# iacopo97/Multimodal-SAM-Adapter

Hardware: AMD Instinct MI355X
Metric: images/sec encoder fwd @1024x1024 RGB+LiDAR ViT-L (higher is better)
Workload: dtype split-operand MFMA: fp16 hi + e5m2 cross terms (h8c / h8 planes, ViT / interaction / up-conv GEMMs) fp16 hi/lo pairs x3 (TwinConvNeXt: f3 planes) and bf16 hi/lo x3 (neck, head); attention blocks with the rel-pos terms fused: every contraction on one fp16 MFMA (q, k, v, P rounded to fp16) in the bloc

## Files before the change

### include/mmsa.h

```cpp
#ifndef MMSA_H
#define MMSA_H
#include <stddef.h>
#include <stdint.h>
#ifdef __cplusplus
extern "C" {
#endif

#ifdef MMSA_BUILDING_LIBRARY
typedef hipStream_t mmsa_stream_t;
#else
typedef void* mmsa_stream_t;
#endif

#include "mmsa_version.h"
int mmsa_version(void);
const char* mmsa_last_error(void);

int mmsa_debug_poison_lds(unsigned pattern, mmsa_stream_t stream);
int mmsa_event_create(void** ev);
int mmsa_event_record(void* ev, mmsa_stream_t stream);
int mmsa_event_elapsed_ms(void* start, void* stop, float* ms);
int mmsa_event_destroy(void* ev);

enum { MMSA_ACT_NONE = 0, MMSA_ACT_GELU = 1, MMSA_ACT_RELU = 2, MMSA_ACT_RELU6 = 3, MMSA_ACT_HSWISH = 4, MMSA_ACT_SIGMOID = 5 };
// ... 16 lines not shown
int mmsa_msda_fused(const float* value, const int64_t* spatial_shapes, const int64_t* level_start_index,
                    const float* raw, long ldraw, const float* ref_points, float* out, long ldo,
                    uint16_t* out_planes, long ldop , int out_fmt , int batch,
                    int spatial_size, int num_heads, int channels, int num_levels, int num_query, int num_point,
                    float* clamp_max , mmsa_stream_t stream);

int mmsa_msda_fused_planes(const uint16_t* value_planes, long ldvp, int lo_bytes, const int64_t* spatial_shapes, const int64_t* level_start_index,
                           const float* raw, long ldraw, const float* ref_points, float* out, long ldo,
                           uint16_t* out_planes, long ldop, int out_fmt, int batch,
                           int spatial_size, int num_heads, int channels, int num_levels, int num_query, int num_point,
                           float* clamp_max, mmsa_stream_t stream);

int mmsa_rowstats_finalize(const float* rowstats, int rows, int strips, int D, float eps, float* mean_rstd, mmsa_stream_t stream);

int mmsa_zero_bytes(void* p, size_t bytes, mmsa_stream_t stream);
int mmsa_gemm_split3(const float* A, const uint16_t* Ap, long lda, long strideA,
                     const uint16_t* Wp, long strideW,
                     const float* bias, long strideBias, const float* colscale, const float* resid, long ldr,
                     long strideR, int resid_mod, float beta, float* C, long ldc, long strideC,
                     uint16_t* Cp, long ldcp, long strideCp, int M, int N, int K,
                     int batch, int act, float alpha, int out_mode, int ps_H, int ps_W, int ps_C, int fmt, int cp_fmt,
                     int max_grid, float* rowstats_out, const float* rownorm_mean_rstd, const float* rownorm_colsum, int flavour,
                     float* clamp_max , mmsa_stream_t stream);

int mmsa_convnext_mlp_fused(const uint16_t* Ap, long lda, long strideA, const uint16_t* W1p, long strideW1, const uint16_t* W2p,
                            long strideW2, const float* b1, const float* b2, const float* gamma, float* x, long ldx, long strideX,
                            int M, int C, int batch, int max_grid, int fmt,
                            float* clamp_max , mmsa_stream_t stream);

int mmsa_split_planes(const float* src, long ld, int rows, int cols, int cols_pad, uint16_t* planes, int kind,
                      float* clamp_max , mmsa_stream_t stream);

int mmsa_attention(const float* qkv, long ldq, const float* qkv_bias, const float* rp, float* out, long ldo, int B,
                   int H, int W, int heads, int head_dim, int window_size, float scale, mmsa_stream_t stream);
int mmsa_attention_planes(const uint16_t* qkv_planes, long ldq, const uint16_t* bias_planes, const float* rp,
                          uint16_t* out_planes, long ldo, int B, int H, int W, int heads, int head_dim,
                          int window_size, float scale, int out_fmt ,
                          int v_fmt ,
                          float* max_abs_logit , mmsa_stream_t stream);

int mmsa_relpos_bias(const float* qkv, long ldq, const float* Rh, const float* Rw, float* rp, int B, int H, int W,
                     int heads, int head_dim, int window_size, mmsa_stream_t stream);
int mmsa_relpos_bias_planes(const uint16_t* qkv_planes, long ldq, const float* Rh, const float* Rw,
                            float* rp, int B, int H, int W, int heads, int head_dim, int window_size, mmsa_stream_t stream);

int mmsa_layernorm_rows(const float* x, long ldx, const float* w, const float* b, float eps, float* y, long ldy,
// ... 108 lines not shown
```

### include/mmsa_version.h

```cpp
#ifndef MMSA_VERSION_H
#define MMSA_VERSION_H
#define MMSA_ABI_VERSION 109
#endif
```

### multimodal-sam-adapter_amd/csrc/gemm_split3.hip

```cpp
#include "common.h"

struct GemmArgs {
  const float* A; const unsigned short* Ap; long lda; long strideA;
  const unsigned short* Wp; long strideW;
  const float* bias; long strideBias;
  const float* colscale;
  const float* resid; long ldr; long strideR; int resid_mod; float beta;
  float* C; long ldc; long strideC;
  unsigned short* Cp; long ldcp; long strideCp;
  int M, N, K;
  int act; float alpha;
  int out_mode; int ps_H, ps_W, ps_C;
  int cp_fmt;
  float* clamp_max;
};

#define BM 128
#define BN 128
#define BK 32
#define PLANE_BYTES (4 * 128 * 16)
#define STAGE_BYTES (4 * PLANE_BYTES)

template <bool AP, bool GEN, bool F16 = false>
__global__ __launch_bounds__(256) void gemm_split3_kernel(GemmArgs a) {
// ... 202 lines not shown
        for (int r = 0; r < 4; ++r) {
          if (n + r < a.N) {
            float x = v[r];
            if (resid) x += a.beta * resid[rrow * a.ldr + dcol + r];
            if (C) C[drow * a.ldc + dcol + r] = x;
            if (Cp) { clamp_see1(cw_, x); store_planes1(Cp + drow * a.ldcp, dcol + r, x, MMSA_CP_AT(a.cp_fmt, dcol + r)); }
          }
        }
      }
    }
  }
  if (Cp) clamp_report(a.clamp_max, cw_, MMSA_CP_SPLIT(a.cp_fmt) ? MMSA_H8_MAX : mmsa_clamp_limit(MMSA_CP_BASE(a.cp_fmt)));
}

int mmsa_gemm_v2_launch(const unsigned short* Ap, long lda, long strideA,
                        const unsigned short* Wp, long strideW,
                        const float* bias, long strideBias, const float* colscale,
                        const float* resid, long ldr, long strideR, int resid_mod, float beta,
                        float* C, long ldc, long strideC,
                        unsigned short* Cp, long ldcp, long strideCp,
                        int M, int N, int K, int batch, int act, float alpha,
                        int out_mode, int ps_H, int ps_W, int ps_C, int fmt, int cp_fmt, int max_grid, hipStream_t stream,
                        float* rs_out, const float* rn_mr, const float* rn_cs, int flavour, float* clamp_max);

__global__ __launch_bounds__(256) void gemm_tiny_kernel(GemmArgs a, int ncg) {
  const int lane = threadIdx.x & 63;
  const long wv = (long)blockIdx.x * 4 + (threadIdx.x >> 6);
  const long per_b = (long)a.M * ncg;
  const int bz = blockIdx.y;
  if (wv >= per_b) return;
  const int m = (int)(wv / ncg), n0 = (int)(wv - (long)m * ncg) * 8;
  const float* A = a.A + (long)bz * a.strideA + (long)m * a.lda;
  const unsigned short* Wp = a.Wp + (long)bz * a.strideW;
  float acc[8];
#pragma unroll
  for (int j = 0; j < 8; ++j) acc[j] = 0.f;
  for (int k = lane * 4; k < a.K; k += 256) {
    const float4 x = *reinterpret_cast<const float4*>(A + k);
    const int ko = ilv(k);
#pragma unroll
    for (int j = 0; j < 8; ++j) {
      const int n = min(n0 + j, a.N - 1);
      const unsigned short* wr = Wp + (long)n * 2 * a.K + ko;
      const uint2 h = *reinterpret_cast<const uint2*>(wr), l = *reinterpret_cast<const uint2*>(wr + 32);
      const float w0 = __uint_as_float(h.x << 16) + __uint_as_float(l.x << 16);
      const float w1 = __uint_as_float(h.x & 0xFFFF0000u) + __uint_as_float(l.x & 0xFFFF0000u);
// ... 71 lines not shown
  a.bias = bias; a.strideBias = strideBias; a.colscale = colscale;
  a.resid = resid; a.ldr = ldr; a.strideR = strideR; a.resid_mod = resid_mod; a.beta = beta;
  a.C = C; a.ldc = C ? ldc : 0; a.strideC = strideC;
  a.Cp = Cp; a.ldcp = Cp ? ldcp : 0; a.strideCp = strideCp;
  a.M = M; a.N = N; a.K = K; a.act = act; a.alpha = alpha;
  a.out_mode = out_mode; a.ps_H = ps_H; a.ps_W = ps_W; a.ps_C = ps_C; a.cp_fmt = cp_fmt;
  a.clamp_max = clamp_max;
  const bool force_v1 = MMSA_KNOB("MMSA_GEMM_V1", 0) != 0;
  const bool narrow = false;
  const bool no_tiny = MMSA_KNOB("MMSA_GEMM_NO_TINY", 0) != 0;
  if (!ap && !Cp && out_mode == 0 && resid_mod <= 0 && (N <= 64 || K <= 64) && M <= 16384 && !no_tiny && !extras && fmt == MMSA_FMT_B3) {
    const int ncg = cdiv(N, 8);
    hipLaunchKernelGGL(gemm_tiny_kernel, dim3(cdiv((long)M * ncg, 4), batch), dim3(256), 0, stream, a, ncg);
    MMSA_CHECK_LAUNCH("gemm_split3(tiny)");
    return MMSA_OK;
  }
  if (ap && (fmt != MMSA_FMT_B3 || (M >= 128 && !force_v1 && !narrow))) {
    return mmsa_gemm_v2_launch(Ap, lda, strideA, Wp, strideW, bias, strideBias, colscale, resid, ldr, strideR,
                               resid_mod, beta, C, ldc, strideC, Cp, ldcp, strideCp, M, N, K, batch, act, alpha,
                               out_mode, ps_H, ps_W, ps_C, fmt, cp_fmt, max_grid, stream, rs_out, rn_mr, rn_cs, flavour, clamp_max);
  }
  MMSA_CHECK_ARG(!extras, "gemm_split3: this shape is not routed to the LDS-DMA kernel, which alone writes row statistics / normalises rows");
  MMSA_CHECK_ARG(!cp_h8c, "gemm_split3: h8c output planes are written by the LDS-DMA kernel only (activation planes in, M >= 128)");
  dim3 grid(cdiv(N, BN), cdiv(M, BM), batch);
  const bool gen = out_mode != 0 || resid_mod > 0;
  if (ap) {
    if (gen) hipLaunchKernelGGL((gemm_split3_kernel<true, true>), grid, dim3(256), 2 * STAGE_BYTES, stream, a);
    else hipLaunchKernelGGL((gemm_split3_kernel<true, false>), grid, dim3(256), 2 * STAGE_BYTES, stream, a);
  } else if (fmt == MMSA_FMT_F3) {
    if (gen) hipLaunchKernelGGL((gemm_split3_kernel<false, true, true>), grid, dim3(256), 2 * STAGE_BYTES, stream, a);
    else hipLaunchKernelGGL((gemm_split3_kernel<false, false, true>), grid, dim3(256), 2 * STAGE_BYTES, stream, a);
  } else {
    if (gen) hipLaunchKernelGGL((gemm_split3_kernel<false, true>), grid, dim3(256), 2 * STAGE_BYTES, stream, a);
    else hipLaunchKernelGGL((gemm_split3_kernel<false, false>), grid, dim3(256), 2 * STAGE_BYTES, stream, a);
  }
  MMSA_CHECK_LAUNCH("gemm_split3");
  return MMSA_OK;
}

__global__ void split_planes_kernel(const float* __restrict__ src, long ld, int rows, int cols, int cols_pad,
                                    unsigned short* __restrict__ out, int kind, float* __restrict__ clamp_max) {
  const long total = (long)rows * cols_pad;
  float cw_ = 0.f;
  for (long i = (long)blockIdx.x * blockDim.x + threadIdx.x; i < total; i += (long)gridDim.x * blockDim.x) {
    const int r = (int)(i / cols_pad), c = (int)(i % cols_pad);
    const float x = c < cols ? src[(long)r * ld + c] : 0.f;
// ... 38 lines not shown
```

### multimodal-sam-adapter_amd/csrc/gemm_stream.hip

```cpp
#include "gemm_v2_shared.h"

struct GemmStreamArgs {
  const unsigned short* Ap; long lda;
  const unsigned short* Wp;
  const float* bias; const float* colscale; float alpha;
  const float* resid; long ldr; float beta;
  float* C; long ldc;
  unsigned short* Cp; long ldcp; int cp_fmt;
  int M, act;
  float* clamp_max;
};

#define GS_WROW(K_) ((K_) * 4 + 16)

template <int NT, int KS, bool F16, bool RES>
__global__ __launch_bounds__(512, 1) void gemm_stream_kernel(GemmStreamArgs a) {
  constexpr int N = NT * 16, K = KS * 32;
  extern __shared__ __attribute__((aligned(16))) unsigned char smem[];
  const int tid = threadIdx.x, lane = tid & 63;
  const int wave = __builtin_amdgcn_readfirstlane(tid >> 6);
  const int l15 = lane & 15, g = lane >> 4;

  {
    constexpr int PIECES = N * KS * 8;
    const unsigned char* wsrc = reinterpret_cast<const unsigned char*>(a.Wp);
    for (int p = tid; p < PIECES; p += 512) {
      const int n = p / (KS * 8), q = p - n * (KS * 8);
      *reinterpret_cast<uint4*>(smem + n * GS_WROW(K) + q * 16) = *reinterpret_cast<const uint4*>(wsrc + (long)n * (K * 4) + q * 16);
    }
  }
  if (tid < N) {
    float* cvl = reinterpret_cast<float*>(smem + N * GS_WROW(K));
    cvl[tid] = a.bias ? a.bias[tid] : 0.f;
    cvl[N + tid] = (a.colscale ? a.colscale[tid] : 1.f) * a.alpha;
  }
  __syncthreads();

  const int nblk = (a.M + 15) >> 4;
  const int stride = gridDim.x * 8;
  int blk = blockIdx.x * 8 + wave;
  if (blk >= nblk) return;
  const unsigned char* Ab = reinterpret_cast<const unsigned char*>(a.Ap);
  const long ldaB = a.lda * 2;
  const unsigned woff0 = (unsigned)(l15 * GS_WROW(K) + g * 16);

  uint4 fa[2][KS][2];
  auto load_block = [&](int b_, uint4 (&f)[KS][2]) {
    const int row = min(b_ * 16 + l15, a.M - 1);
    const unsigned char* rp = Ab + (long)row * ldaB + g * 16;
#pragma unroll
    for (int ks = 0; ks < KS; ++ks) {
      f[ks][0] = *reinterpret_cast<const uint4*>(rp + ks * 128);
      f[ks][1] = *reinterpret_cast<const uint4*>(rp + ks * 128 + 64);
    }
  };
  const int cp_base = MMSA_CP_BASE(a.cp_fmt);
  const bool act_on = a.act != ACT_NONE;
  const float act_hi = a.act == ACT_RELU6 ? 6.0f : INFINITY;
  float cw_ = 0.f;
  const float* colv = reinterpret_cast<const float*>(smem + N * GS_WROW(K)) + 4 * g;

  auto compute_store = [&](int b_, const uint4 (&f)[KS][2]) {
    const int m = b_ * 16 + l15;
    float4 rr[NT];
    if constexpr (RES) {
      const float* rrow = a.resid + (long)min(m, a.M - 1) * a.ldr + 4 * g;
#pragma unroll
      for (int nt = 0; nt < NT; ++nt) rr[nt] = *reinterpret_cast<const float4*>(rrow + nt * 16);
    }
    f32x4 acc[NT];
#pragma unroll
    for (int nt = 0; nt < NT; ++nt) acc[nt] = (f32x4){0.f, 0.f, 0.f, 0.f};
    unsigned woff = woff0;
    asm volatile("" : "+v"(woff));
    const unsigned char* wl_ = smem + woff;
#pragma unroll
    for (int ks = 0; ks < KS; ++ks) {
#pragma unroll
      for (int nt = 0; nt < NT; ++nt) {
        const uint4 wh = *reinterpret_cast<const uint4*>(wl_ + nt * 16 * GS_WROW(K) + ks * 128);
        const uint4 wl = *reinterpret_cast<const uint4*>(wl_ + nt * 16 * GS_WROW(K) + ks * 128 + 64);
        if constexpr (F16) {
          acc[nt] = __builtin_amdgcn_mfma_f32_16x16x32_f16(__builtin_bit_cast(f16x8, wl), __builtin_bit_cast(f16x8, f[ks][0]), acc[nt], 0, 0, 0);
          acc[nt] = __builtin_amdgcn_mfma_f32_16x16x32_f16(__builtin_bit_cast(f16x8, wh), __builtin_bit_cast(f16x8, f[ks][1]), acc[nt], 0, 0, 0);
          acc[nt] = __builtin_amdgcn_mfma_f32_16x16x32_f16(__builtin_bit_cast(f16x8, wh), __builtin_bit_cast(f16x8, f[ks][0]), acc[nt], 0, 0, 0);
        } else {
          acc[nt] = __builtin_amdgcn_mfma_f32_16x16x32_bf16(__builtin_bit_cast(bf16x8, wl), __builtin_bit_cast(bf16x8, f[ks][0]), acc[nt], 0, 0, 0);
          acc[nt] = __builtin_amdgcn_mfma_f32_16x16x32_bf16(__builtin_bit_cast(bf16x8, wh), __builtin_bit_cast(bf16x8, f[ks][1]), acc[nt], 0, 0, 0);
          acc[nt] = __builtin_amdgcn_mfma_f32_16x16x32_bf16(__builtin_bit_cast(bf16x8, wh), __builtin_bit_cast(bf16x8, f[ks][0]), acc[nt], 0, 0, 0);
        }
      }
    }
    if (m < a.M) {
#pragma unroll
      for (int nt = 0; nt < NT; ++nt) {
        const int n = nt * 16 + 4 * g;
        const float4 bv = *reinterpret_cast<const float4*>(colv + 16 * nt), cv = *reinterpret_cast<const float4*>(colv + N + 16 * nt);
        float4 o = make_float4(acc[nt][0] + bv.x, acc[nt][1] + bv.y, acc[nt][2] + bv.z, acc[nt][3] + bv.w);
        if (act_on) { o.x = fminf(fmaxf(o.x, 0.0f), act_hi); o.y = fminf(fmaxf(o.y, 0.0f), act_hi); o.z = fminf(fmaxf(o.z, 0.0f), act_hi); o.w = fminf(fmaxf(o.w, 0.0f), act_hi); }
        o.x *= cv.x; o.y *= cv.y; o.z *= cv.z; o.w *= cv.w;
        if constexpr (RES) { o.x += a.beta * rr[nt].x; o.y += a.beta * rr[nt].y; o.z += a.beta * rr[nt].z; o.w += a.beta * rr[nt].w; }
        if (a.C) *reinterpret_cast<float4*>(a.C + (long)m * a.ldc + n) = o;
        if (a.Cp) {
          clamp_see(cw_, o);
          store_planes4(a.Cp + (long)m * a.ldcp, n, o, cp_base);
        }
      }
    }
  };

  const int lastb = nblk - 1;
  load_block(blk, fa[0]);
#pragma unroll 1
  for (;;) {
    const int nb1 = blk + stride;
    load_block(min(nb1, lastb), fa[1]);
    compute_store(blk, fa[0]);
    if (nb1 >= nblk) break;
    const int nb2 = nb1 + stride;
    load_block(min(nb2, lastb), fa[0]);
    compute_store(nb1, fa[1]);
    if (nb2 >= nblk) break;
    blk = nb2;
  }
  if (a.Cp) clamp_report(a.clamp_max, cw_, mmsa_clamp_limit(cp_base));
}

int mmsa_gemm_stream_try(const unsigned short* Ap, long lda, const unsigned short* Wp, const float* bias, const float* colscale, const float* resid, long ldr, float beta,
                         float* C, long ldc, unsigned short* Cp, long ldcp, int M, int N, int K, int batch, int act, float alpha, int out_mode, int resid_mod,
                         int fmt, int cp_fmt, int max_grid, const float* rs_out, const float* rn_mr, int flavour, float* clamp_max, hipStream_t stream) {
#ifndef MMSA_GEMM_STREAM_DEFAULT
#define MMSA_GEMM_STREAM_DEFAULT 1
#endif
  if (MMSA_KNOB("MMSA_GEMM_STREAM", MMSA_GEMM_STREAM_DEFAULT) == 0 || flavour != 0) return 0;
  if (!(fmt == MMSA_FMT_B3 || fmt == MMSA_FMT_F3) || batch != 1 || out_mode != 0 || resid_mod > 0 || rs_out || rn_mr) return 0;
  if (!((N == 96 && K == 192) || (N == 192 && K == 96)) || M < 16384) return 0;
  if (!(act == ACT_NONE || act == ACT_RELU || act == ACT_RELU6)) return 0;
  if (Cp && (MMSA_CP_SPLIT(cp_fmt) != 0 || !(MMSA_CP_BASE(cp_fmt) == MMSA_FMT_B3 || MMSA_CP_BASE(cp_fmt) == MMSA_FMT_F3))) return 0;
  const uintptr_t al = (uintptr_t)Ap | (uintptr_t)Wp | (uintptr_t)bias | (uintptr_t)colscale | (uintptr_t)resid | (uintptr_t)C | (uintptr_t)Cp;
  if ((al & 15) || (lda & 7) || (C && (ldc & 3)) || (resid && (ldr & 3)) || (Cp && (ldcp & 7)) || lda < 2L * K || (Cp && ldcp < 2L * N)) return 0;
  GemmStreamArgs a;
  a.Ap = Ap; a.lda = lda; a.Wp = Wp; a.bias = bias; a.colscale = colscale; a.alpha = alpha; a.resid = resid; a.ldr = ldr; a.beta = beta;
  a.C = C; a.ldc = ldc; a.Cp = Cp; a.ldcp = ldcp; a.cp_fmt = cp_fmt; a.M = M; a.act = act; a.clamp_max = clamp_max;
  static MmsaPerDevice per_dev_ = {};
  const int num_cus = mmsa_per_device(per_dev_, [] {
#define GS_ATTR(NT_, KS_, F_) (void)hipFuncSetAttribute((const void*)gemm_stream_kernel<NT_, KS_, F_, false>, hipFuncAttributeMaxDynamicSharedMemorySize, (NT_) * 16 * GS_WROW((KS_) * 32) + (NT_) * 16 * 8); \
                              (void)hipFuncSetAttribute((const void*)gemm_stream_kernel<NT_, KS_, F_, true>, hipFuncAttributeMaxDynamicSharedMemorySize, (NT_) * 16 * GS_WROW((KS_) * 32) + (NT_) * 16 * 8);
    GS_ATTR(6, 6, false) GS_ATTR(6, 6, true) GS_ATTR(12, 3, false) GS_ATTR(12, 3, true)
#undef GS_ATTR
  });
  const int cus = (max_grid > 0 && max_grid < num_cus) ? max_grid : num_cus;
  const int nblk = (M + 15) / 16;
  const int grid = nblk / 8 < cus ? (nblk + 7) / 8 : cus;
  const int lds = N * GS_WROW(K) + N * 8;
  const bool f16 = fmt == MMSA_FMT_F3;
#define GS_LAUNCH(NT_, KS_)                                                                                                   \
  { if (f16 && resid) hipLaunchKernelGGL((gemm_stream_kernel<NT_, KS_, true, true>), dim3(grid), dim3(512), lds, stream, a);      \
    else if (f16) hipLaunchKernelGGL((gemm_stream_kernel<NT_, KS_, true, false>), dim3(grid), dim3(512), lds, stream, a);          \
    else if (resid) hipLaunchKernelGGL((gemm_stream_kernel<NT_, KS_, false, true>), dim3(grid), dim3(512), lds, stream, a);        \
    else hipLaunchKernelGGL((gemm_stream_kernel<NT_, KS_, false, false>), dim3(grid), dim3(512), lds, stream, a); }
  if (N == 96 && K == 192) GS_LAUNCH(6, 6)
  else GS_LAUNCH(12, 3)
#undef GS_LAUNCH
  MMSA_CHECK_LAUNCH("gemm_split3(stream)");
  return 1;
}
```

### multimodal-sam-adapter_amd/csrc/gemm_v2.hip

```cpp
#include "common.h"
#include "gemm_v2_shared.h"
template <bool GEN, int ACT, bool PP, int NW, int FMT>
__global__ __launch_bounds__(NW * 64, NW == 4 ? 2 : 1) void gemm_v2_kernel(GemmV2Args a) {
  static_assert(NW == 8 || (NW == 4 && !PP), "4-wave workgroups run the in-phase main loop");
  static_assert(FMT == MMSA_FMT_B3 || (PP && NW == 8), "the h8 and f3 operand formats run on the ping-pong kernel");
  constexpr bool EPI_UNROLL = ACT >= 0;
  constexpr int V2_BM = NW * 32;
  constexpr int V2_A_BYTES = V2_BM * 128;
  constexpr int V2_STAGE = V2_A_BYTES + V2_W_BYTES;
  constexpr int V2_NST = NW == 8 ? 3 : 2;
  constexpr int WROWS = V2_BN / NW;
  constexpr int NDMA = 4 + WROWS / 8;
  extern __shared__ __attribute__((aligned(16))) unsigned char smem[];
  const int tid = threadIdx.x;
  const int lane = tid & 63;
  const int wave = __builtin_amdgcn_readfirstlane(tid >> 6);
  const int wm = wave >> 1, wn = wave & 1;
  const int grp = wave >> 2;
  const int l15 = lane & 15, g = lane >> 4;
  const int K = a.K;
  const int nk = K / V2_BK;

  const int G = gridDim.x;
  int rb = blockIdx.x;
// ... 403 lines not shown
    const int st_cur = st == 0 ? V2_NST - 1 : st - 1;

    if (V2_DBG(a) == 2 || V2_DBG(a) == 5 || V2_DBG(a) >= 64) { tile += G; continue; }
#define EPI_STAGING_BASE (smem + st_cur * V2_STAGE)
#include "gemm_v2_epilogue.inc"
    if constexpr (PP) {
      asm volatile("s_waitcnt lgkmcnt(0)" ::: "memory");
      __builtin_amdgcn_s_barrier();
    }
    tile += G;
  }
  CLK_SAMPLE(2)
#undef K_STEP
#undef K_STEP_PP
#undef K_STEP_PP_FAST
#undef PP_WAIT
#undef PP_PIECE
#undef MFMA_CHUNK
#undef MFMA_FP8_ALL
}

int mmsa_gemm_h8c_dispatch(const GemmV2Args& a, int grid, bool gen, int act, hipStream_t stream);
int mmsa_gemm_h8c_w8_dispatch(const GemmV2Args& a, int grid, bool gen, int act, hipStream_t stream);
int mmsa_gemm_stream_try(const unsigned short* Ap, long lda, const unsigned short* Wp, const float* bias, const float* colscale, const float* resid, long ldr, float beta,
                         float* C, long ldc, unsigned short* Cp, long ldcp, int M, int N, int K, int batch, int act, float alpha, int out_mode, int resid_mod,
                         int fmt, int cp_fmt, int max_grid, const float* rs_out, const float* rn_mr, int flavour, float* clamp_max, hipStream_t stream);
int mmsa_gemm_h8c4_dispatch(const GemmV2Args& a, int grid, hipStream_t stream);

int mmsa_gemm_v2_launch(const unsigned short* Ap, long lda, long strideA,
                        const unsigned short* Wp, long strideW,
                        const float* bias, long strideBias, const float* colscale,
                        const float* resid, long ldr, long strideR, int resid_mod, float beta,
                        float* C, long ldc, long strideC,
                        unsigned short* Cp, long ldcp, long strideCp,
                        int M, int N, int K, int batch, int act, float alpha,
                        int out_mode, int ps_H, int ps_W, int ps_C, int fmt, int cp_fmt, int max_grid, hipStream_t stream,
                        float* rs_out, const float* rn_mr, const float* rn_cs, int flavour, float* clamp_max) {
  {
    const int rc_ = mmsa_gemm_stream_try(Ap, lda, Wp, bias, colscale, resid, ldr, beta, C, ldc, Cp, ldcp, M, N, K, batch, act, alpha, out_mode, resid_mod, fmt, cp_fmt,
                                         max_grid, rs_out, rn_mr, flavour, clamp_max, stream);
    if (rc_ != 0) return rc_ < 0 ? rc_ : MMSA_OK;
  }
  GemmV2Args a;
  a.clamp_max = clamp_max;
  MMSA_CHECK_ARG(!rs_out || (C && out_mode == 0 && resid_mod <= 0 && act == ACT_NONE && (N & 63) == 0 && (ldc & 3) == 0 && (!resid || (ldr & 3) == 0) && (!Cp || (ldcp & 3) == 0)),
                 "gemm(v2): row statistics need a plain fp32 output, no activation, N %% 64 == 0 (N=%d)", N);
  MMSA_CHECK_ARG(!rn_mr || (rn_cs && !resid && out_mode == 0 && resid_mod <= 0 && (N & 127) == 0 && ((((uintptr_t)bias) | ((uintptr_t)colscale) | ((uintptr_t)rn_cs)) & 15) == 0 && (strideBias & 3) == 0 &&
                            ((Cp && !C && (act == ACT_NONE || act == ACT_GELU || act == ACT_RELU)) ||
                             (C && !Cp && act == ACT_NONE && (M & 255) == 0 && !colscale && alpha == 1.0f && (ldc & 3) == 0 && (((uintptr_t)C) & 15) == 0))),
                 "gemm(v2): the row-normalising epilogue needs N %% 128 == 0 (N=%d), 16-byte aligned column vectors and either a planes-only output or a plain fp32 output with M %% 256 == 0 (M=%d), no activation / scale", N, M);
  a.rs_out = rs_out; a.rs_strips = N >> 6; a.rn_mr = rn_mr; a.rn_cs = rn_cs;
  a.Ap = Ap; a.lda = lda; a.strideA = strideA;
  a.Wp = Wp; a.strideW = strideW;
  const bool w8 = fmt == MMSA_FMT_W8;
  const bool h8c = fmt == MMSA_FMT_H8C || w8;
  MMSA_CHECK_ARG(!w8 || ((K & 127) == 0 && batch == 1), "gemm(v2): W8 weights need K %% 128 == 0 and one batch (K=%d, batch=%d)", K, batch);
  a.ldw = w8 ? K / 2 : h8c ? 3L * K : 2L * K;
  a.bias = bias; a.strideBias = strideBias; a.colscale = colscale;
  a.resid = resid; a.ldr = ldr; a.strideR = strideR; a.resid_mod = resid_mod; a.beta = beta;
  a.C = C; a.ldc = C ? ldc : 0; a.strideC = strideC;
  a.Cp = Cp; a.ldcp = Cp ? ldcp : 0; a.strideCp = strideCp;
  a.M = M; a.N = N; a.K = K; a.act = act; a.alpha = alpha;
  a.out_mode = out_mode; a.ps_H = ps_H; a.ps_W = ps_W; a.ps_C = ps_C;
  auto log2_exact = [](int v) { int s_ = -1; if (v > 0 && (v & (v - 1)) == 0) { s_ = 0; while ((1 << s_) < v) ++s_; } return s_; };
  a.ps_sw = log2_exact(ps_W); a.ps_sh = log2_exact(ps_H);
// ... 79 lines not shown
```

### multimodal-sam-adapter_amd/mmsa/lib.py

```python
import ctypes
import os
from ctypes import c_char_p, c_double, c_float, c_int, c_long, c_void_p, POINTER

_HERE = os.path.dirname(os.path.abspath(__file__))
LIB_PATH = os.environ.get("MMSA_LIB") or os.path.join(_HERE, "libmmsa_hip.so")

if not os.path.exists(LIB_PATH):
    raise RuntimeError(
        f"{LIB_PATH} not found: the MI355X HIP library is required (no CPU/PyTorch fallback exists). "
        "Build it with: python multimodal-sam-adapter_amd/build.py")

import torch

_lib = ctypes.CDLL(LIB_PATH)

P = c_void_p
I = c_int
L = c_long
F = c_float

SIGNATURES = {
    "mmsa_version": [],
    "mmsa_last_error": [],
    "mmsa_debug_poison_lds": [ctypes.c_uint, P],
    "mmsa_event_create": [POINTER(c_void_p)],
    "mmsa_event_record": [P, P],
    "mmsa_event_elapsed_ms": [P, P, POINTER(c_float)],
    "mmsa_event_destroy": [P],
    "mmsa_ms_deform_attn_forward": [P, P, P, P, P, P, I, I, I, I, I, I, I, I, I, P],
    "mmsa_ms_deform_attn_backward": [P, P, P, P, P, P, P, P, P, I, I, I, I, I, I, I, I, I, P],
    "mmsa_msda_fused": [P, P, P, P, L, P, P, L, P, L, I, I, I, I, I, I, I, I, P, P],
    "mmsa_msda_fused_planes": [P, L, I, P, P, P, L, P, P, L, P, L, I, I, I, I, I, I, I, I, P, P],
    "mmsa_gemm_split3": [P, P, L, L, P, L, P, L, P, P, L, L, I, F, P, L, L, P, L, L, I, I, I, I, I, F, I, I, I, I, I, I, I, P, P, P, I, P, P],
    "mmsa_convnext_mlp_fused": [P, L, L, P, L, P, L, P, P, P, P, L, L, I, I, I, I, I, P, P],
    "mmsa_rowstats_finalize": [P, I, I, I, F, P, P],
    "mmsa_zero_bytes": [P, ctypes.c_size_t, P],
    "mmsa_split_planes": [P, L, I, I, I, P, I, P, P],
    "mmsa_attention": [P, L, P, P, P, L, I, I, I, I, I, I, F, P],
    "mmsa_attention_planes": [P, L, P, P, P, L, I, I, I, I, I, I, F, I, I, P, P],
    "mmsa_relpos_bias": [P, L, P, P, P, I, I, I, I, I, I, P],
    "mmsa_relpos_bias_planes": [P, L, P, P, P, I, I, I, I, I, I, P],
    "mmsa_layernorm_rows": [P, L, P, P, F, P, L, P, L, P, L, I, I, I, I, I, I, L, L, I, I, P, P],
    "mmsa_colstats": [P, L, L, P, I, I, I, P, I, P],
    "mmsa_ffrm_finalize": [P, I, I, I, F, F, P, P, P, P, P, P, P, P],
    "mmsa_lnhw_apply": [P, L, P, P, P, P, P, P, L, I, I, I, P],
    "mmsa_dwconv_nhwc": [P, L, L, P, P, P, L, L, P, L, L, I, I, I, I, I, I, I, I, P, P, P],
    "mmsa_dwpair_gate": [P, L, P, P, L, P, L, I, I, I, I, P],
    "mmsa_gconv_nhwc": [P, L, P, P, P, L, I, I, I, I, I, I, I, I, P],
    "mmsa_gfe_qkv_conv": [P, L, P, P, L, I, I, I, I, I, I, POINTER(c_int), P],
    "mmsa_im2col_nchw": [P, I, I, I, I, I, I, I, P, I, P],
    "mmsa_gram_tn": [P, L, P, L, L, P, I, I, I, I, P, L, P],
    "mmsa_gram_tn_scratch_bytes": [I, I, I],
    "mmsa_chanattn_build": [P, P, L, P, L, P, P, P, I, I, I, I, P],
    "mmsa_gffm_build": [P, P, P, I, I, I, P],
    "mmsa_gelu_gate": [P, L, P, L, L, I, P],
    "mmsa_pool_hw": [P, L, P, L, I, I, I, I, P],
# ... 7 lines not shown
    "mmsa_bilinear_accum_nchw": [P, L, I, I, I, I, P, I, I, I, I, I, I, P, I, P],
    "mmsa_div_count_nchw": [P, P, I, I, L, P],
    "mmsa_argmax_nchw": [P, P, I, I, L, P],
    "mmsa_crop_batch_nchw": [P, I, I, I, I, P, I, P, I, I, P],
    "mmsa_slide_argmax": [P, I, I, I, I, P, P, I, I, I, I, I, P, P],
    "mmsa_slide_argmax_resized": [P, I, I, I, I, P, P, I, I, I, I, I, I, I, I, I, P, P],
    "mmsa_preprocess_nhwc": [P, I, P, I, I, I, I, P, P, P, P, P, P, I, I, P],
    "mmsa_preprocess_crops": [P, I, P, I, I, I, I, P, P, P, P, P, I, I, P, I, P, I, I, P],
    "mmsa_preprocess_resize_nhwc": [P, I, P, I, I, I, I, P, P, P, P, P, P, I, I, I, I, P, P, P, P, I, P],
    "mmsa_preprocess_resize_crops": [P, I, P, I, I, I, I, P, P, P, P, P, I, I, P, I, P, I, I, I, I, P, P, P, P, I, P],
    "mmsa_eval_confusion_u8": [P, P, I, I, I, I, I, P, I, P, P, P, I, P, P],
    "mmsa_slide_argmax_eval": [P, I, I, I, I, P, P, I, I, I, I, I, P, P, I, I, P, P, P, P, I, P, P],
    "mmsa_render_u8": [P, L, L, I, I, I, P, I, I, P, I, I, I, c_double, c_double, P, P],
    "mmsa_render_denorm_f32": [P, L, L, I, I, I, P, I, I, P, I, I, I, P, P, I, I, c_double, c_double, P, P],
}
_RESTYPES = {"mmsa_last_error": c_char_p, "mmsa_gram_tn_scratch_bytes": c_long}

for _name, _args in SIGNATURES.items():
    _fn = getattr(_lib, _name)
    _fn.argtypes = _args
    _fn.restype = _RESTYPES.get(_name, c_int)


ABI_VERSION = 109
if _lib.mmsa_version() != ABI_VERSION:
    raise RuntimeError(f"{LIB_PATH}: ABI version {_lib.mmsa_version()} but mmsa/lib.py binds version {ABI_VERSION} (include/mmsa.h MMSA_ABI_VERSION): "
                       "rebuild with python multimodal-sam-adapter_amd/build.py")


def last_error() -> str:
    return _lib.mmsa_last_error().decode()


POISON_LDS = os.environ.get("MMSA_DEBUG_POISON_LDS") == "1"


def call(name, *args):
    if POISON_LDS and not name.startswith(("mmsa_event", "mmsa_debug")) and args:
        _lib.mmsa_debug_poison_lds(0x7FC07FC0, args[-1])
    rc = getattr(_lib, name)(*args)
    if rc != 0:
        raise RuntimeError(f"{name} failed (rc={rc}): {last_error()}")


def version() -> int:
    return _lib.mmsa_version()

# ... 3 lines not shown
```

Measured before the change: 66.98.

## Generalise streaming GEMM to more shapes, batches, fp32 A input and GELU epilogue

Extends the weight-stationary streaming GEMM kernel to a table of extra (N,K) shapes, with batched operands, column chunking across blocks (XCD remap), fp32 A input split on the fly into hi/lo planes, and a fused GELU epilogue. The fp32-A path is also tried from the v1 gemm_split3 route, so low-arithmetic-intensity GEMMs avoid the tiled kernel and any separate plane-splitting pass. A flop/byte gate keeps compute-heavy shapes on the old kernels. This adds template instantiations and a routing query exported to Python, at the risk of lower occupancy or poor chunking on some shapes.

```diff
diff --git a/include/mmsa.h b/include/mmsa.h
--- a/include/mmsa.h
+++ b/include/mmsa.h
@@ -62,6 +62,7 @@
                      int batch, int act, float alpha, int out_mode, int ps_H, int ps_W, int ps_C, int fmt, int cp_fmt,
                      int max_grid, float* rowstats_out, const float* rownorm_mean_rstd, const float* rownorm_colsum, int flavour,
                      float* clamp_max , mmsa_stream_t stream);
+int mmsa_gemm_stream_routes(int a_fp32, int M, int N, int K, int batch, int act, int has_resid, int has_c, int has_cp, int fmt, int cp_fmt, int flavour);
 
 int mmsa_convnext_mlp_fused(const uint16_t* Ap, long lda, long strideA, const uint16_t* W1p, long strideW1, const uint16_t* W2p,
                             long strideW2, const float* b1, const float* b2, const float* gamma, float* x, long ldx, long strideX,
diff --git a/include/mmsa_version.h b/include/mmsa_version.h
--- a/include/mmsa_version.h
+++ b/include/mmsa_version.h
@@ -1,4 +1,4 @@
 #ifndef MMSA_VERSION_H
 #define MMSA_VERSION_H
-#define MMSA_ABI_VERSION 109
+#define MMSA_ABI_VERSION 110
 #endif
diff --git a/multimodal-sam-adapter_amd/csrc/gemm_split3.hip b/multimodal-sam-adapter_amd/csrc/gemm_split3.hip
--- a/multimodal-sam-adapter_amd/csrc/gemm_split3.hip
+++ b/multimodal-sam-adapter_amd/csrc/gemm_split3.hip
@@ -248,6 +248,10 @@
                         int M, int N, int K, int batch, int act, float alpha,
                         int out_mode, int ps_H, int ps_W, int ps_C, int fmt, int cp_fmt, int max_grid, hipStream_t stream,
                         float* rs_out, const float* rn_mr, const float* rn_cs, int flavour, float* clamp_max);
+int mmsa_gemm_stream_try(const float* A, const unsigned short* Ap, long lda, long strideA, const unsigned short* Wp, long strideW, const float* bias, long strideBias,
+                         const float* colscale, const float* resid, long ldr, long strideR, float beta, float* C, long ldc, long strideC,
+                         unsigned short* Cp, long ldcp, long strideCp, int M, int N, int K, int batch, int act, float alpha, int out_mode, int resid_mod,
+                         int fmt, int cp_fmt, int max_grid, const float* rs_out, const float* rn_mr, int flavour, float* clamp_max, hipStream_t stream);
 
 __global__ __launch_bounds__(256) void gemm_tiny_kernel(GemmArgs a, int ncg) {
   const int lane = threadIdx.x & 63;
@@ -365,6 +369,11 @@
   }
   MMSA_CHECK_ARG(!extras, "gemm_split3: this shape is not routed to the LDS-DMA kernel, which alone writes row statistics / normalises rows");
   MMSA_CHECK_ARG(!cp_h8c, "gemm_split3: h8c output planes are written by the LDS-DMA kernel only (activation planes in, M >= 128)");
+  if (!ap) {
+    const int rc_ = mmsa_gemm_stream_try(A, nullptr, lda, strideA, Wp, strideW, bias, strideBias, colscale, resid, ldr, strideR, beta, C, ldc, strideC, Cp, ldcp, strideCp,
+                                         M, N, K, batch, act, alpha, out_mode, resid_mod, fmt, cp_fmt, max_grid, rs_out, rn_mr, flavour, clamp_max, stream);
+    if (rc_ != 0) return rc_ < 0 ? rc_ : MMSA_OK;
+  }
   dim3 grid(cdiv(N, BN), cdiv(M, BM), batch);
   const bool gen = out_mode != 0 || resid_mod > 0;
   if (ap) {
diff --git a/multimodal-sam-adapter_amd/csrc/gemm_stream.hip b/multimodal-sam-adapter_amd/csrc/gemm_stream.hip
--- a/multimodal-sam-adapter_amd/csrc/gemm_stream.hip
+++ b/multimodal-sam-adapter_amd/csrc/gemm_stream.hip
@@ -1,29 +1,37 @@
 #include "gemm_v2_shared.h"
 
 struct GemmStreamArgs {
-  const unsigned short* Ap; long lda;
-  const unsigned short* Wp;
-  const float* bias; const float* colscale; float alpha;
-  const float* resid; long ldr; float beta;
-  float* C; long ldc;
-  unsigned short* Cp; long ldcp; int cp_fmt;
+  const void* Ap; long lda; long strideA;
+  const unsigned short* Wp; long strideW;
+  const float* bias; const float* colscale; long strideBias; float alpha;
+  const float* resid; long ldr; long strideR; float beta;
+  float* C; long ldc; long strideC;
+  unsigned short* Cp; long ldcp; long strideCp; int cp_fmt;
   int M, act;
+  int nch, batch;
   float* clamp_max;
 };
 
 #define GS_WROW(K_) ((K_) * 4 + 16)
 
-template <int NT, int KS, bool F16, bool RES>
+template <int NT, int KS, bool F16, int EPI, bool A32>
 __global__ __launch_bounds__(512, 1) void gemm_stream_kernel(GemmStreamArgs a) {
   constexpr int N = NT * 16, K = KS * 32;
+  constexpr bool RES = EPI == 1;
   extern __shared__ __attribute__((aligned(16))) unsigned char smem[];
   const int tid = threadIdx.x, lane = tid & 63;
   const int wave = __builtin_amdgcn_readfirstlane(tid >> 6);
   const int l15 = lane & 15, g = lane >> 4;
+  int rb = blockIdx.x;
+  if (a.nch > 1) V2_XCD_REMAP(rb, (int)gridDim.x)
+  const int gq = rb / a.nch, chunk = rb - gq * a.nch;
+  const int gi = gq / a.batch, bz = gq - gi * a.batch;
+  const int GB = gridDim.x / (a.nch * a.batch);
+  const int ncol0 = chunk * N;
 
   {
     constexpr int PIECES = N * KS * 8;
-    const unsigned char* wsrc = reinterpret_cast<const unsigned char*>(a.Wp);
+    const unsigned char* wsrc = reinterpret_cast<const unsigned char*>(a.Wp + (long)bz * a.strideW) + (long)ncol0 * (K * 4);
     for (int p = tid; p < PIECES; p += 512) {
       const int n = p / (KS * 8), q = p - n * (KS * 8);
       *reinterpret_cast<uint4*>(smem + n * GS_WROW(K) + q * 16) = *reinterpret_cast<const uint4*>(wsrc + (long)n * (K * 4) + q * 16);
@@ -31,27 +39,32 @@
   }
   if (tid < N) {
     float* cvl = reinterpret_cast<float*>(smem + N * GS_WROW(K));
-    cvl[tid] = a.bias ? a.bias[tid] : 0.f;
-    cvl[N + tid] = (a.colscale ? a.colscale[tid] : 1.f) * a.alpha;
+    const long cvo = (long)bz * a.strideBias + ncol0 + tid;
+    cvl[tid] = a.bias ? a.bias[cvo] : 0.f;
+    cvl[N + tid] = (a.colscale ? a.colscale[cvo] : 1.f) * a.alpha;
   }
   __syncthreads();
 
   const int nblk = (a.M + 15) >> 4;
-  const int stride = gridDim.x * 8;
-  int blk = blockIdx.x * 8 + wave;
+  const int stride = GB * 8;
+  int blk = gi * 8 + wave;
   if (blk >= nblk) return;
-  const unsigned char* Ab = reinterpret_cast<const unsigned char*>(a.Ap);
-  const long ldaB = a.lda * 2;
+  constexpr int AEL = A32 ? 4 : 2;
+  const unsigned char* Ab = reinterpret_cast<const unsigned char*>(a.Ap) + (long)bz * a.strideA * AEL;
+  const long ldaB = a.lda * AEL;
+  const float* residb = RES ? a.resid + (long)bz * a.strideR : nullptr;
+  float* Cb = a.C ? a.C + (long)bz * a.strideC : nullptr;
+  unsigned short* Cpb = a.Cp ? a.Cp + (long)bz * a.strideCp : nullptr;
   const unsigned woff0 = (unsigned)(l15 * GS_WROW(K) + g * 16);
 
   uint4 fa[2][KS][2];
   auto load_block = [&](int b_, uint4 (&f)[KS][2]) {
     const int row = min(b_ * 16 + l15, a.M - 1);
-    const unsigned char* rp = Ab + (long)row * ldaB + g * 16;
+    const unsigned char* rp = Ab + (long)row * ldaB + g * (A32 ? 32 : 16);
 #pragma unroll
     for (int ks = 0; ks < KS; ++ks) {
       f[ks][0] = *reinterpret_cast<const uint4*>(rp + ks * 128);
-      f[ks][1] = *reinterpret_cast<const uint4*>(rp + ks * 128 + 64);
+      f[ks][1] = *reinterpret_cast<const uint4*>(rp + ks * 128 + (A32 ? 16 : 64));
     }
   };
   const int cp_base = MMSA_CP_BASE(a.cp_fmt);
@@ -64,7 +77,7 @@
     const int m = b_ * 16 + l15;
     float4 rr[NT];
     if constexpr (RES) {
-      const float* rrow = a.resid + (long)min(m, a.M - 1) * a.ldr + 4 * g;
+      const float* rrow = residb + (long)min(m, a.M - 1) * a.ldr + ncol0 + 4 * g;
 #pragma unroll
       for (int nt = 0; nt < NT; ++nt) rr[nt] = *reinterpret_cast<const float4*>(rrow + nt * 16);
     }
@@ -76,34 +89,43 @@
     const unsigned char* wl_ = smem + woff;
 #pragma unroll
     for (int ks = 0; ks < KS; ++ks) {
+      uint4 ah_ = f[ks][0], al_ = f[ks][1];
+      if constexpr (A32) {
+        uint2 h0, l0, h1, l1;
+        const float4 v0 = __builtin_bit_cast(float4, f[ks][0]), v1 = __builtin_bit_cast(float4, f[ks][1]);
+        if constexpr (F16) { f3_split4(v0, h0, l0); f3_split4(v1, h1, l1); } else { split4(v0, h0, l0); split4(v1, h1, l1); }
+        ah_ = make_uint4(h0.x, h0.y, h1.x, h1.y);
+        al_ = make_uint4(l0.x, l0.y, l1.x, l1.y);
+      }
 #pragma unroll
       for (int nt = 0; nt < NT; ++nt) {
         const uint4 wh = *reinterpret_cast<const uint4*>(wl_ + nt * 16 * GS_WROW(K) + ks * 128);
         const uint4 wl = *reinterpret_cast<const uint4*>(wl_ + nt * 16 * GS_WROW(K) + ks * 128 + 64);
         if constexpr (F16) {
-          acc[nt] = __builtin_amdgcn_mfma_f32_16x16x32_f16(__builtin_bit_cast(f16x8, wl), __builtin_bit_cast(f16x8, f[ks][0]), acc[nt], 0, 0, 0);
-          acc[nt] = __builtin_amdgcn_mfma_f32_16x16x32_f16(__builtin_bit_cast(f16x8, wh), __builtin_bit_cast(f16x8, f[ks][1]), acc[nt], 0, 0, 0);
-          acc[nt] = __builtin_amdgcn_mfma_f32_16x16x32_f16(__builtin_bit_cast(f16x8, wh), __builtin_bit_cast(f16x8, f[ks][0]), acc[nt], 0, 0, 0);
+          acc[nt] = __builtin_amdgcn_mfma_f32_16x16x32_f16(__builtin_bit_cast(f16x8, wl), __builtin_bit_cast(f16x8, ah_), acc[nt], 0, 0, 0);
+          acc[nt] = __builtin_amdgcn_mfma_f32_16x16x32_f16(__builtin_bit_cast(f16x8, wh), __builtin_bit_cast(f16x8, al_), acc[nt], 0, 0, 0);
+          acc[nt] = __builtin_amdgcn_mfma_f32_16x16x32_f16(__builtin_bit_cast(f16x8, wh), __builtin_bit_cast(f16x8, ah_), acc[nt], 0, 0, 0);
         } else {
-          acc[nt] = __builtin_amdgcn_mfma_f32_16x16x32_bf16(__builtin_bit_cast(bf16x8, wl), __builtin_bit_cast(bf16x8, f[ks][0]), acc[nt], 0, 0, 0);
-          acc[nt] = __builtin_amdgcn_mfma_f32_16x16x32_bf16(__builtin_bit_cast(bf16x8, wh), __builtin_bit_cast(bf16x8, f[ks][1]), acc[nt], 0, 0, 0);
-          acc[nt] = __builtin_amdgcn_mfma_f32_16x16x32_bf16(__builtin_bit_cast(bf16x8, wh), __builtin_bit_cast(bf16x8, f[ks][0]), acc[nt], 0, 0, 0);
+          acc[nt] = __builtin_amdgcn_mfma_f32_16x16x32_bf16(__builtin_bit_cast(bf16x8, wl), __builtin_bit_cast(bf16x8, ah_), acc[nt], 0, 0, 0);
+          acc[nt] = __builtin_amdgcn_mfma_f32_16x16x32_bf16(__builtin_bit_cast(bf16x8, wh), __builtin_bit_cast(bf16x8, al_), acc[nt], 0, 0, 0);
+          acc[nt] = __builtin_amdgcn_mfma_f32_16x16x32_bf16(__builtin_bit_cast(bf16x8, wh), __builtin_bit_cast(bf16x8, ah_), acc[nt], 0, 0, 0);
         }
       }
     }
     if (m < a.M) {
 #pragma unroll
       for (int nt = 0; nt < NT; ++nt) {
-        const int n = nt * 16 + 4 * g;
+        const int n = ncol0 + nt * 16 + 4 * g;
         const float4 bv = *reinterpret_cast<const float4*>(colv + 16 * nt), cv = *reinterpret_cast<const float4*>(colv + N + 16 * nt);
         float4 o = make_float4(acc[nt][0] + bv.x, acc[nt][1] + bv.y, acc[nt][2] + bv.z, acc[nt][3] + bv.w);
-        if (act_on) { o.x = fminf(fmaxf(o.x, 0.0f), act_hi); o.y = fminf(fmaxf(o.y, 0.0f), act_hi); o.z = fminf(fmaxf(o.z, 0.0f), act_hi); o.w = fminf(fmaxf(o.w, 0.0f), act_hi); }
+        if constexpr (EPI == 2) o = gelu4(o);
+        else if (act_on) { o.x = fminf(fmaxf(o.x, 0.0f), act_hi); o.y = fminf(fmaxf(o.y, 0.0f), act_hi); o.z = fminf(fmaxf(o.z, 0.0f), act_hi); o.w = fminf(fmaxf(o.w, 0.0f), act_hi); }
         o.x *= cv.x; o.y *= cv.y; o.z *= cv.z; o.w *= cv.w;
         if constexpr (RES) { o.x += a.beta * rr[nt].x; o.y += a.beta * rr[nt].y; o.z += a.beta * rr[nt].z; o.w += a.beta * rr[nt].w; }
-        if (a.C) *reinterpret_cast<float4*>(a.C + (long)m * a.ldc + n) = o;
-        if (a.Cp) {
+        if (Cb) *reinterpret_cast<float4*>(Cb + (long)m * a.ldc + n) = o;
+        if (Cpb) {
           clamp_see(cw_, o);
-          store_planes4(a.Cp + (long)m * a.ldcp, n, o, cp_base);
+          store_planes4(Cpb + (long)m * a.ldcp, n, o, cp_base);
         }
       }
     }
@@ -126,42 +148,93 @@
   if (a.Cp) clamp_report(a.clamp_max, cw_, mmsa_clamp_limit(cp_base));
 }
 
-int mmsa_gemm_stream_try(const unsigned short* Ap, long lda, const unsigned short* Wp, const float* bias, const float* colscale, const float* resid, long ldr, float beta,
-                         float* C, long ldc, unsigned short* Cp, long ldcp, int M, int N, int K, int batch, int act, float alpha, int out_mode, int resid_mod,
-                         int fmt, int cp_fmt, int max_grid, const float* rs_out, const float* rn_mr, int flavour, float* clamp_max, hipStream_t stream) {
+struct GsShape { int N, K; bool a32; int NT; bool by_default; long max_rows; };
+static const GsShape GS_SHAPES[] = {
+  {96, 192, false, 6, true, 0},    {192, 96, false, 12, true, 0},
+  {768, 192, false, 12, true, 0},  {1024, 192, false, 8, true, 0},  {384, 192, false, 12, true, 65536},
+  {192, 192, false, 6, false, 0},  {96, 96, false, 6, false, 0},
+  {96, 64, true, 6, true, 0},      {96, 96, true, 6, true, 0},      {192, 192, true, 6, true, 0},
+};
+static const GsShape* gs_shape(int N, int K, bool a32) {
+  for (const GsShape& s : GS_SHAPES) if (s.N == N && s.K == K && s.a32 == a32) return &s;
+  return nullptr;
+}
+static const GsShape* gs_routes(int a32, int M, int N, int K, int batch, int act, int has_resid, int has_c, int has_cp, int out_mode, int resid_mod, int fmt, int cp_fmt, int flavour) {
 #ifndef MMSA_GEMM_STREAM_DEFAULT
 #define MMSA_GEMM_STREAM_DEFAULT 1
 #endif
-  if (MMSA_KNOB("MMSA_GEMM_STREAM", MMSA_GEMM_STREAM_DEFAULT) == 0 || flavour != 0) return 0;
-  if (!(fmt == MMSA_FMT_B3 || fmt == MMSA_FMT_F3) || batch != 1 || out_mode != 0 || resid_mod > 0 || rs_out || rn_mr) return 0;
-  if (!((N == 96 && K == 192) || (N == 192 && K == 96)) || M < 16384) return 0;
-  if (!(act == ACT_NONE || act == ACT_RELU || act == ACT_RELU6)) return 0;
-  if (Cp && (MMSA_CP_SPLIT(cp_fmt) != 0 || !(MMSA_CP_BASE(cp_fmt) == MMSA_FMT_B3 || MMSA_CP_BASE(cp_fmt) == MMSA_FMT_F3))) return 0;
-  const uintptr_t al = (uintptr_t)Ap | (uintptr_t)Wp | (uintptr_t)bias | (uintptr_t)colscale | (uintptr_t)resid | (uintptr_t)C | (uintptr_t)Cp;
-  if ((al & 15) || (lda & 7) || (C && (ldc & 3)) || (resid && (ldr & 3)) || (Cp && (ldcp & 7)) || lda < 2L * K || (Cp && ldcp < 2L * N)) return 0;
+  if (MMSA_KNOB("MMSA_GEMM_STREAM", MMSA_GEMM_STREAM_DEFAULT) == 0 || !(flavour == 0 || flavour == 1)) return nullptr;
+  if (!(fmt == MMSA_FMT_B3 || fmt == MMSA_FMT_F3) || batch < 1 || batch > 8 || out_mode != 0 || resid_mod > 0 || M < 1) return nullptr;
+#ifndef MMSA_GEMM_STREAM_WIDE
+#define MMSA_GEMM_STREAM_WIDE 1
+#endif
+  const GsShape* s = gs_shape(N, K, a32 != 0);
+  if (!MMSA_GEMM_STREAM_WIDE && flavour == 0 && (a32 || batch != 1 || !((N == 96 && K == 192) || (N == 192 && K == 96)))) return nullptr;
+  const long rows = (long)M * batch;
+  if (!s || (flavour == 0 && (!s->by_default || rows < 16384 || (s->max_rows > 0 && rows > s->max_rows)))) return nullptr;
+  if (!(act == ACT_NONE || act == ACT_RELU || act == ACT_RELU6 || (act == ACT_GELU && !has_resid && !a32))) return nullptr;
+  if (has_cp && (MMSA_CP_SPLIT(cp_fmt) != 0 || !(MMSA_CP_BASE(cp_fmt) == MMSA_FMT_B3 || MMSA_CP_BASE(cp_fmt) == MMSA_FMT_F3))) return nullptr;
+  const double flop = 2.0 * M * N * K, bytes = 4.0 * ((double)M * K + (double)N * K) + 4.0 * M * N * ((has_c ? 1 : 0) + (has_cp ? 1 : 0) + (has_resid ? 1 : 0));
+  if (flop >= 100.0 * bytes) return nullptr;
+  return s;
+}
+extern "C" int mmsa_gemm_stream_routes(int a_fp32, int M, int N, int K, int batch, int act, int has_resid, int has_c, int has_cp, int fmt, int cp_fmt, int flavour) {
+  return gs_routes(a_fp32, M, N, K, batch, act, has_resid, has_c, has_cp, 0, 0, fmt, cp_fmt, flavour) ? 1 : 0;
+}
+
+int mmsa_gemm_stream_try(const float* A, const unsigned short* Ap, long lda, long strideA, const unsigned short* Wp, long strideW, const float* bias, long strideBias,
+                         const float* colscale, const float* resid, long ldr, long strideR, float beta, float* C, long ldc, long strideC,
+                         unsigned short* Cp, long ldcp, long strideCp, int M, int N, int K, int batch, int act, float alpha, int out_mode, int resid_mod,
+                         int fmt, int cp_fmt, int max_grid, const float* rs_out, const float* rn_mr, int flavour, float* clamp_max, hipStream_t stream) {
+  const bool a32 = A != nullptr;
+  if (rs_out || rn_mr) return 0;
+  const GsShape* sh = gs_routes(a32, M, N, K, batch, act, resid != nullptr, C != nullptr, Cp != nullptr, out_mode, resid_mod, fmt, cp_fmt, flavour);
+  if (!sh) return 0;
+  const uintptr_t al = (uintptr_t)A | (uintptr_t)Ap | (uintptr_t)Wp | (uintptr_t)bias | (uintptr_t)colscale | (uintptr_t)resid | (uintptr_t)C | (uintptr_t)Cp;
+  const long am = a32 ? 3 : 7, kmin = a32 ? K : 2L * K;
+  if ((al & 15) || (lda & am) || (strideA & am) || (strideW & 7) || (strideBias & 3) || (C && ((ldc | strideC) & 3)) || (resid && ((ldr | strideR) & 3)) ||
+      (Cp && ((ldcp | strideCp) & 7)) || lda < kmin || (Cp && ldcp < 2L * N) || (C && ldc < N) || (resid && ldr < N)) return 0;
   GemmStreamArgs a;
-  a.Ap = Ap; a.lda = lda; a.Wp = Wp; a.bias = bias; a.colscale = colscale; a.alpha = alpha; a.resid = resid; a.ldr = ldr; a.beta = beta;
-  a.C = C; a.ldc = ldc; a.Cp = Cp; a.ldcp = ldcp; a.cp_fmt = cp_fmt; a.M = M; a.act = act; a.clamp_max = clamp_max;
+  a.Ap = a32 ? (const void*)A : (const void*)Ap; a.lda = lda; a.strideA = strideA; a.Wp = Wp; a.strideW = strideW;
+  a.bias = bias; a.colscale = colscale; a.strideBias = strideBias; a.alpha = alpha; a.resid = resid; a.ldr = ldr; a.strideR = strideR; a.beta = beta;
+  a.C = C; a.ldc = ldc; a.strideC = strideC; a.Cp = Cp; a.ldcp = ldcp; a.strideCp = strideCp; a.cp_fmt = cp_fmt; a.M = M; a.act = act; a.clamp_max = clamp_max;
+  const int NC = sh->NT * 16;
+  a.nch = N / NC; a.batch = batch;
+#define GS_TABLE(X_) X_(6, 6, false, false, true) X_(12, 3, false, false, true) X_(12, 6, false, true, false) X_(8, 6, false, false, true) X_(6, 3, false, false, true) \
+                     X_(6, 2, true, false, true) X_(6, 3, true, false, true) X_(6, 6, true, false, true)
+#define GS_LDS(NT_, KS_) ((NT_) * 16 * GS_WROW((KS_) * 32) + (NT_) * 16 * 8)
   static MmsaPerDevice per_dev_ = {};
   const int num_cus = mmsa_per_device(per_dev_, [] {
-#define GS_ATTR(NT_, KS_, F_) (void)hipFuncSetAttribute((const void*)gemm_stream_kernel<NT_, KS_, F_, false>, hipFuncAttributeMaxDynamicSharedMemorySize, (NT_) * 16 * GS_WROW((KS_) * 32) + (NT_) * 16 * 8); \
-                              (void)hipFuncSetAttribute((const void*)gemm_stream_kernel<NT_, KS_, F_, true>, hipFuncAttributeMaxDynamicSharedMemorySize, (NT_) * 16 * GS_WROW((KS_) * 32) + (NT_) * 16 * 8);
-    GS_ATTR(6, 6, false) GS_ATTR(6, 6, true) GS_ATTR(12, 3, false) GS_ATTR(12, 3, true)
+#define GS_ATTR1(NT_, KS_, F_, E_, A32_) (void)hipFuncSetAttribute((const void*)gemm_stream_kernel<NT_, KS_, F_, E_, A32_>, hipFuncAttributeMaxDynamicSharedMemorySize, GS_LDS(NT_, KS_));
+#define GS_ATTR(NT_, KS_, A32_, G_, R_) GS_ATTR1(NT_, KS_, false, 0, A32_) GS_ATTR1(NT_, KS_, true, 0, A32_) \
+                                    if (R_) { GS_ATTR1(NT_, KS_, false, (R_) ? 1 : 0, A32_) GS_ATTR1(NT_, KS_, true, (R_) ? 1 : 0, A32_) } \
+                                    if (G_) { GS_ATTR1(NT_, KS_, false, (G_) ? 2 : 0, A32_) GS_ATTR1(NT_, KS_, true, (G_) ? 2 : 0, A32_) }
+    GS_TABLE(GS_ATTR)
 #undef GS_ATTR
+#undef GS_ATTR1
   });
   const int cus = (max_grid > 0 && max_grid < num_cus) ? max_grid : num_cus;
   const int nblk = (M + 15) / 16;
-  const int grid = nblk / 8 < cus ? (nblk + 7) / 8 : cus;
-  const int lds = N * GS_WROW(K) + N * 8;
+  int gb = cus / (a.nch * batch);
+  if (gb < 1) return 0;
+  if ((nblk + 7) / 8 < gb) gb = (nblk + 7) / 8;
+  const int grid = gb * batch * a.nch;
   const bool f16 = fmt == MMSA_FMT_F3;
-#define GS_LAUNCH(NT_, KS_)                                                                                                   \
-  { if (f16 && resid) hipLaunchKernelGGL((gemm_stream_kernel<NT_, KS_, true, true>), dim3(grid), dim3(512), lds, stream, a);      \
-    else if (f16) hipLaunchKernelGGL((gemm_stream_kernel<NT_, KS_, true, false>), dim3(grid), dim3(512), lds, stream, a);          \
-    else if (resid) hipLaunchKernelGGL((gemm_stream_kernel<NT_, KS_, false, true>), dim3(grid), dim3(512), lds, stream, a);        \
-    else hipLaunchKernelGGL((gemm_stream_kernel<NT_, KS_, false, false>), dim3(grid), dim3(512), lds, stream, a); }
-  if (N == 96 && K == 192) GS_LAUNCH(6, 6)
-  else GS_LAUNCH(12, 3)
+  const int epi = act == ACT_GELU ? 2 : resid ? 1 : 0;
+  bool launched = false;
+#define GS_LAUNCH1(NT_, KS_, F_, E_, A32_) { hipLaunchKernelGGL((gemm_stream_kernel<NT_, KS_, F_, E_, A32_>), dim3(grid), dim3(512), GS_LDS(NT_, KS_), stream, a); launched = true; }
+#define GS_LAUNCH(NT_, KS_, A32_, G_, R_)                                               \
+  if (!launched && sh->NT == (NT_) && K == (KS_) * 32 && a32 == (A32_)) {               \
+    if (epi == 2) { if (G_) { if (f16) GS_LAUNCH1(NT_, KS_, true, (G_) ? 2 : 0, A32_) else GS_LAUNCH1(NT_, KS_, false, (G_) ? 2 : 0, A32_) } }  \
+    else if (epi == 1) { if (R_) { if (f16) GS_LAUNCH1(NT_, KS_, true, (R_) ? 1 : 0, A32_) else GS_LAUNCH1(NT_, KS_, false, (R_) ? 1 : 0, A32_) } }  \
+    else if (f16) GS_LAUNCH1(NT_, KS_, true, 0, A32_)                                   \
+    else GS_LAUNCH1(NT_, KS_, false, 0, A32_)                                           \
+  }
+  GS_TABLE(GS_LAUNCH)
 #undef GS_LAUNCH
+#undef GS_LAUNCH1
+#undef GS_TABLE
+  if (!launched) return 0;
   MMSA_CHECK_LAUNCH("gemm_split3(stream)");
   return 1;
 }
diff --git a/multimodal-sam-adapter_amd/csrc/gemm_v2.hip b/multimodal-sam-adapter_amd/csrc/gemm_v2.hip
--- a/multimodal-sam-adapter_amd/csrc/gemm_v2.hip
+++ b/multimodal-sam-adapter_amd/csrc/gemm_v2.hip
@@ -449,8 +449,9 @@
 
 int mmsa_gemm_h8c_dispatch(const GemmV2Args& a, int grid, bool gen, int act, hipStream_t stream);
 int mmsa_gemm_h8c_w8_dispatch(const GemmV2Args& a, int grid, bool gen, int act, hipStream_t stream);
-int mmsa_gemm_stream_try(const unsigned short* Ap, long lda, const unsigned short* Wp, const float* bias, const float* colscale, const float* resid, long ldr, float beta,
-                         float* C, long ldc, unsigned short* Cp, long ldcp, int M, int N, int K, int batch, int act, float alpha, int out_mode, int resid_mod,
+int mmsa_gemm_stream_try(const float* A, const unsigned short* Ap, long lda, long strideA, const unsigned short* Wp, long strideW, const float* bias, long strideBias,
+                         const float* colscale, const float* resid, long ldr, long strideR, float beta, float* C, long ldc, long strideC,
+                         unsigned short* Cp, long ldcp, long strideCp, int M, int N, int K, int batch, int act, float alpha, int out_mode, int resid_mod,
                          int fmt, int cp_fmt, int max_grid, const float* rs_out, const float* rn_mr, int flavour, float* clamp_max, hipStream_t stream);
 int mmsa_gemm_h8c4_dispatch(const GemmV2Args& a, int grid, hipStream_t stream);
 
@@ -464,10 +465,11 @@
                         int out_mode, int ps_H, int ps_W, int ps_C, int fmt, int cp_fmt, int max_grid, hipStream_t stream,
                         float* rs_out, const float* rn_mr, const float* rn_cs, int flavour, float* clamp_max) {
   {
-    const int rc_ = mmsa_gemm_stream_try(Ap, lda, Wp, bias, colscale, resid, ldr, beta, C, ldc, Cp, ldcp, M, N, K, batch, act, alpha, out_mode, resid_mod, fmt, cp_fmt,
-                                         max_grid, rs_out, rn_mr, flavour, clamp_max, stream);
+    const int rc_ = mmsa_gemm_stream_try(nullptr, Ap, lda, strideA, Wp, strideW, bias, strideBias, colscale, resid, ldr, strideR, beta, C, ldc, strideC, Cp, ldcp, strideCp,
+                                         M, N, K, batch, act, alpha, out_mode, resid_mod, fmt, cp_fmt, max_grid, rs_out, rn_mr, flavour, clamp_max, stream);
     if (rc_ != 0) return rc_ < 0 ? rc_ : MMSA_OK;
   }
+  if (flavour == 1) flavour = 0;
   GemmV2Args a;
   a.clamp_max = clamp_max;
   MMSA_CHECK_ARG(!rs_out || (C && out_mode == 0 && resid_mod <= 0 && act == ACT_NONE && (N & 63) == 0 && (ldc & 3) == 0 && (!resid || (ldr & 3) == 0) && (!Cp || (ldcp & 3) == 0)),
diff --git a/multimodal-sam-adapter_amd/mmsa/lib.py b/multimodal-sam-adapter_amd/mmsa/lib.py
--- a/multimodal-sam-adapter_amd/mmsa/lib.py
+++ b/multimodal-sam-adapter_amd/mmsa/lib.py
@@ -32,6 +32,7 @@
     "mmsa_msda_fused": [P, P, P, P, L, P, P, L, P, L, I, I, I, I, I, I, I, I, P, P],
     "mmsa_msda_fused_planes": [P, L, I, P, P, P, L, P, P, L, P, L, I, I, I, I, I, I, I, I, P, P],
     "mmsa_gemm_split3": [P, P, L, L, P, L, P, L, P, P, L, L, I, F, P, L, L, P, L, L, I, I, I, I, I, F, I, I, I, I, I, I, I, P, P, P, I, P, P],
+    "mmsa_gemm_stream_routes": [I, I, I, I, I, I, I, I, I, I, I, I],
     "mmsa_convnext_mlp_fused": [P, L, L, P, L, P, L, P, P, P, P, L, L, I, I, I, I, I, P, P],
     "mmsa_rowstats_finalize": [P, I, I, I, F, P, P],
     "mmsa_zero_bytes": [P, ctypes.c_size_t, P],
@@ -85,7 +86,7 @@
     _fn.restype = _RESTYPES.get(_name, c_int)
 
 
-ABI_VERSION = 109
+ABI_VERSION = 110
 if _lib.mmsa_version() != ABI_VERSION:
     raise RuntimeError(f"{LIB_PATH}: ABI version {_lib.mmsa_version()} but mmsa/lib.py binds version {ABI_VERSION} (include/mmsa.h MMSA_ABI_VERSION): "
                        "rebuild with python multimodal-sam-adapter_amd/build.py")
```

New measurement: 67.24, median of 6. Within noise of the previous version (+0.4%).
